# prs-eth/PCAccumulation

Measured on AMD Instinct MI355X. Metric: LiDAR-frames/sec (5-frame seq, 160k pts) fwd+bwd, higher is better.
Workload: dtype mixed

## Files before the change

include/pcacc.h:

```cpp
#ifndef PCACC_H_
#define PCACC_H_

#include <stddef.h>
#include <stdint.h>

#ifdef __cplusplus
extern "C" {
#endif

#define PCACC_OK 0
#define PCACC_E_ARG (-1)
#define PCACC_E_WORKSPACE (-2)
#define PCACC_E_LAUNCH (-3)

#define PCACC_F32 0
#define PCACC_BF16 1

const char *pcacc_target(void);

int pcacc_cat2_rows(const void *a, int32_t a_row_bytes, const void *b, int32_t b_row_bytes, int64_t rows, void *out, void *stream);

int pcacc_reload_switches(void);

int pcacc_voxelize_workspace_bytes(int64_t n, int nx, int ny, int nz, int nt, size_t *bytes );
// ... 278 lines not shown
                              float *db, int32_t n_img, int32_t frames, int32_t dt, int32_t h, int32_t w, int32_t c_in, int32_t c_out,
                              void *workspace, size_t workspace_bytes, void *stream);
int pcacc_upconv2x2_split_prepare_weights(const float *w, int32_t c_in, int32_t c_up, const int64_t *strides , uint16_t *out_fwd,
                                          float *scale_fwd, uint16_t *out_bwd, float *scale_bwd, void *stream);
int pcacc_upconv2x2_split_supported(int32_t h, int32_t w, int32_t c_in, int32_t c_up);

int pcacc_upconv2x2_bf16_supported(int32_t c_in, int32_t c_up);
int pcacc_upconv2x2_bf16_prepare_weights(const float *w, int32_t c_in, int32_t c_up, const int64_t *strides , uint16_t *out_fwd,
                                         uint16_t *out_bwd, void *stream);
int pcacc_upconv2x2_bf16(const uint16_t *in, const uint16_t *wp, const float *bias, uint16_t *out, int32_t n_img, int32_t h, int32_t w,
                         int32_t c_in, int32_t c_up, int32_t direction, int32_t in_pitch, int32_t out_pitch, void *stream);
int pcacc_upconv2x2_bf16_wgrad_workspace_bytes(int32_t n_img, int32_t h, int32_t w, int32_t c_in, int32_t c_up, size_t *bytes);
int pcacc_upconv2x2_bf16_wgrad(const uint16_t *dy, int32_t dy_pitch, const uint16_t *x, int32_t x_pitch, float *dw, const int64_t *dw_strides ,
                               float *db, int32_t n_img, int32_t h, int32_t w, int32_t c_in, int32_t c_up, void *workspace, size_t workspace_bytes,
                               void *stream);

int pcacc_prepare_weights_batch(const int64_t *jobs, int32_t n_jobs, int32_t total_blocks, void *stream);
int pcacc_upconv2x2_split(const float *in, const float *in_amax, const uint16_t *wp, const float *wscale, const float *bias, float *out,
                          float *out_amax, int32_t n_img, int32_t h, int32_t w, int32_t c_in, int32_t c_up, int32_t direction, void *stream);
int pcacc_upconv2x2_split_dual(const float *in, const float *in_amax, const uint16_t *wp, const float *wscale, const float *bias, float *out,
                               float *out_amax, uint16_t *out16, int32_t n_img, int32_t h, int32_t w, int32_t c_in, int32_t c_up,
                               int32_t out_pitch, void *stream);
int pcacc_upconv2x2_wgrad_split_workspace_bytes(int32_t n_img, int32_t h, int32_t w, int32_t c_in, int32_t c_up, size_t *bytes );
int pcacc_upconv2x2_wgrad_split(const float *dy, const float *dy_amax, const float *x, const float *x_amax, float *dw, float *db4, int32_t n_img,
                                int32_t h, int32_t w, int32_t c_in, int32_t c_up, void *workspace, size_t workspace_bytes, void *stream);
int pcacc_head_conv3x3_supported(int32_t c_in, int32_t c_out);
int pcacc_head_conv3x3_forward(const void *x, int32_t x_dtype, const float *w, const int64_t *w_strides , const float *bias, float *y,
                               int32_t n_img, int32_t h, int32_t wd, int32_t c_in, int32_t c_out, void *stream);
int pcacc_head_conv3x3_dgrad(const float *dy, const float *w, const int64_t *w_strides , void *dx, int32_t dx_dtype, int32_t n_img,
                             int32_t h, int32_t wd, int32_t c_in, int32_t c_out, void *stream);
int pcacc_head_conv3x3_wgrad_workspace_bytes(int32_t n_img, int32_t h, int32_t wd, int32_t c_in, int32_t c_out, size_t *bytes );
int pcacc_head_conv3x3_wgrad(const float *dy, const void *x, int32_t x_dtype, float *dw, float *db, int32_t n_img, int32_t h, int32_t wd,
                             int32_t c_in, int32_t c_out, void *workspace, size_t workspace_bytes, void *stream);
int pcacc_rows_linear_split(const float *x, const float *x_amax, const float *in_mask, const float *w, const float *bias,
                            const float *residual, const float *out_mask, float *y, float *y_amax, int64_t rows, int32_t k, int32_t n,
                            int32_t flags, void *stream);
int pcacc_rows_linear_split_dual(const float *x, const float *x_amax, const float *in_mask, const float *w, const float *bias,
                                 const float *residual, const float *out_mask, float *y, uint16_t *y16, float *y_amax, int64_t rows, int32_t k,
                                 int32_t n, int32_t flags, void *stream);
int pcacc_rows_linear_cat_split(const float *xa, const float *xa_amax, const float *xb, const float *xb_amax, const int32_t *b_index,
                                int32_t ka, const float *in_mask, const float *w, const float *bias, const float *residual,
                                const float *out_mask_a, const float *out_mask_b, float *y, float *y2, int32_t na, float *y_amax, int64_t rows,
                                int32_t k, int32_t n, int32_t flags, void *stream);
int pcacc_rows_wgrad_split_workspace_bytes(int64_t rows, int32_t k, int32_t n, size_t *bytes );
int pcacc_rows_wgrad_split(const float *dy, const float *dy_amax, const float *dy_mask, const float *x, const float *x_amax, int32_t x_relu,
                           int64_t rows, int32_t k, int32_t n, float *dw_aug, void *workspace, size_t workspace_bytes, void *stream);
int pcacc_rows_wgrad_cat_split(const float *dy, const float *dy_amax, const float *dy_mask, const float *xa, const float *xa_amax,
                               const float *xb, const float *xb_amax, const int32_t *b_index, int32_t ka, int32_t x_relu, int64_t rows,
                               int32_t k, int32_t n, float *dw_aug, void *workspace, size_t workspace_bytes, void *stream);
int pcacc_conv3x3_wgrad_workspace_bytes(int32_t n_img, int32_t h, int32_t w, int32_t c_in, int32_t c_out, size_t *bytes );
int pcacc_conv3x3_wgrad_bf16(const uint16_t *dy, const uint16_t *x, float *dw, int32_t n_img, int32_t frames, int32_t dt,
                             int32_t h, int32_t w, int32_t c_in, int32_t c_out, void *workspace, size_t workspace_bytes,
                             void *stream);

int pcacc_prep_points(const double *points, const double *tsfm12, const double *noise, double noise_scale, double scale,
                      double crop_xy, double z_min, double z_max, int32_t remove_ground, double ground_z, int64_t m,
                      double *out_points, uint8_t *keep, void *stream);

int pcacc_seg_loss_workspace_bytes(int64_t n, size_t *bytes );
int pcacc_seg_loss_forward(const void *logits, int logits_dtype, int64_t plane, const int64_t *labels, const int64_t *rows,
                           int64_t n, float *out_loss, double *out_metric, float *lovasz_grad, float *saved,
                           void *workspace, size_t workspace_bytes, void *stream);
int pcacc_seg_loss_backward(const void *logits, int logits_dtype, int64_t plane, const int64_t *labels, const int64_t *rows,
                            int64_t n, int64_t n_total, const float *lovasz_grad, const float *saved, const float *grad_bce,
                            const float *grad_lovasz, void *grad_logits, void *stream);

int pcacc_offset_loss_workspace_bytes(int64_t m, int64_t k, size_t *bytes );
int pcacc_offset_loss_forward(const float *points, const int64_t *time_indice, const int64_t *inst_labels,
                              const int64_t *label_base, const float *ego_motion, const float *inst_motion, int32_t n_frames,
                              int64_t n, int64_t k, const float *transformed_points, const float *offset_est,
                              const int64_t *rows, int64_t m, float *out, float *offset_gt, void *workspace,
                              size_t workspace_bytes, void *stream);
int pcacc_offset_loss_backward(const float *offset_gt, const float *offset_est, const int64_t *rows, int64_t m, int64_t n,
                               const float *grad_norm, const float *grad_dir, float *grad_est, void *stream);

int pcacc_frames_max(const void *x, int dtype, int64_t n_seq, int32_t frames, int64_t plane, void *out, uint8_t *arg, void *stream);
int pcacc_frames_max_backward(const void *grad_out, const uint8_t *arg, int dtype, int64_t n_seq, int32_t frames, int64_t plane,
                              void *grad_x, void *stream);

int pcacc_bn_rows_workspace_bytes(int64_t rows, int32_t c, size_t *bytes );
int pcacc_bn_rows_forward(const void *x, int dtype, int64_t rows, int32_t c, const float *gamma, const float *beta, float eps,
                          float momentum, float *running_mean, float *running_var, void *y, float *save_mean,
                          float *save_invstd, void *workspace, size_t workspace_bytes, void *stream);
int pcacc_bn_rows_backward(const void *grad_y, const void *x, int dtype, int64_t rows, int32_t c, const float *gamma,
                           const float *save_mean, const float *save_invstd, void *grad_x, float *grad_gamma, float *grad_beta,
                           void *workspace, size_t workspace_bytes, void *stream);

int pcacc_bn_relu_rows_forward(const void *x, int dtype, int64_t rows, int32_t c, const float *gamma, const float *beta, float eps,
                               float momentum, float *running_mean, float *running_var, void *y, float *save_mean, float *save_invstd,
                               void *workspace, size_t workspace_bytes, void *stream);
int pcacc_bn_relu_rows_backward(const void *grad_y, const void *x, int dtype, int64_t rows, int32_t c, const float *gamma, const float *beta,
                                const float *save_mean, const float *save_invstd, void *grad_x, float *grad_gamma, float *grad_beta,
                                void *workspace, size_t workspace_bytes, void *stream);
int pcacc_bn_rows_forward_dual(const float *x, int64_t rows, int32_t c, const float *gamma, const float *beta, float eps, float momentum,
                               float *running_mean, float *running_var, int32_t relu, float *y, uint16_t *y16, float *y_amax, float *save_mean,
                               float *save_invstd, void *workspace, size_t workspace_bytes, void *stream);

int pcacc_bn_rows_backward_m(const void *grad_y, const void *x, int dtype, int64_t rows, int32_t c, const float *gamma, const float *beta,
                             int32_t relu, const float *save_mean, const float *save_invstd, void *grad_x, float *grad_x_amax, float *grad_gamma,
                             float *grad_beta, void *workspace, size_t workspace_bytes, void *stream);

int pcacc_pfn_block_forward(const uint16_t *xa, const uint16_t *pooled, const int32_t *p2v, const float *w0, const float *b0,
                            const float *ws, const float *w1, const float *b1, uint16_t *out, uint16_t *relu_h, int64_t rows, void *stream);
int pcacc_pfn_block_backward_workspace_bytes(int64_t rows, size_t *bytes );
int pcacc_pfn_block_backward(const uint16_t *xa, const uint16_t *pooled, const int32_t *p2v, const uint16_t *relu_h,
                             const uint16_t *grad_out, const float *w0, const float *ws, const float *w1, uint16_t *grad_xa,
// ... 58 lines not shown
```

pcaccumulation_amd/csrc/conv.hip:

```cpp
#include "common.h"

#define CV_TH 8
#define CV_TW 32
#define CV_PW (CV_TW + 2)
#define CV_PH (CV_TH + 2)
#define CV_THREADS 256

__global__ __launch_bounds__(256) void conv_prepare_weights_kernel(const float *__restrict__ w, int o, int i, int kt, int transpose,
                                                                   uint16_t *__restrict__ out)
{
    const int taps = kt * 9;
    const int64_t total = (int64_t)taps * o * i;
    for (int64_t e = (int64_t)blockIdx.x * 256 + threadIdx.x; e < total; e += (int64_t)gridDim.x * 256) {
        const int op = transpose ? i : o, ip = transpose ? o : i;
        const int ci = (int)(e % ip);
        const int co = (int)((e / ip) % op);
        const int tap = (int)(e / ((int64_t)ip * op));
        const int src_tap = transpose ? (taps - 1 - tap) : tap;
        const int so = transpose ? ci : co, si = transpose ? co : ci;
        out[e] = f32_to_bf16(w[((int64_t)so * i + si) * taps + src_tap]);
    }
}

extern "C" int pcacc_conv3x3_prepare_weights(const float *w, int32_t c_out, int32_t c_in, int32_t kt, int32_t transpose,
                                             uint16_t *out, void *stream)
{
    if (!w || !out || c_out < 1 || c_in < 1 || (kt != 1 && kt != 3)) return PCACC_E_ARG;
    const int64_t total = (int64_t)kt * 9 * c_out * c_in;
    hipLaunchKernelGGL(conv_prepare_weights_kernel, dim3(pcacc_grid(total, 256)), dim3(256), 0, pcacc_stream(stream), w, c_out, c_in,
                       kt, transpose, out);
    PCACC_CHECK_LAUNCH();
    return 0;
}

struct ConvWStrides { int64_t o, i, t, y, x; };

__global__ __launch_bounds__(256) void conv_prepare_weights_pair_kernel(const float *__restrict__ w, int o, int i, int kt, ConvWStrides st,
                                                                        uint16_t *__restrict__ out_fwd, uint16_t *__restrict__ out_bwd)
{
    const int taps = kt * 9;
    const int64_t total = (int64_t)taps * o * i;
    for (int64_t e = (int64_t)blockIdx.x * 256 + threadIdx.x; e < 2 * total; e += (int64_t)gridDim.x * 256) {
        const bool transpose = e >= total;
        const int64_t r = transpose ? e - total : e;
        const int op = transpose ? i : o, ip = transpose ? o : i;
        const int ci = (int)(r % ip);
        const int co = (int)((r / ip) % op);
        const int tap = (int)(r / ((int64_t)ip * op));
        const int src_tap = transpose ? (taps - 1 - tap) : tap;
        const int so = transpose ? ci : co, si = transpose ? co : ci;
        const int ft = src_tap / 9, fy = (src_tap % 9) / 3, fx = src_tap % 3;
        const uint16_t v = f32_to_bf16(w[so * st.o + si * st.i + ft * st.t + fy * st.y + fx * st.x]);
        (transpose ? out_bwd : out_fwd)[r] = v;
// ... 617 lines not shown
                const int tap = grp + j * TG;
                if (tap < 9) {
                    const uint16_t *pb = sx + ((ry + tap / 3) * CV_PW + xb + tap % 3 + tr_row) * XS + it * 32 + tr_col;
                    cv_frag bf;
                    bf.h[0] = __builtin_amdgcn_ds_read_tr16_b64_v4i16((pcacc_s16x4 __attribute__((address_space(3))) *)pb);
                    bf.h[1] = __builtin_amdgcn_ds_read_tr16_b64_v4i16((pcacc_s16x4 __attribute__((address_space(3))) *)(pb + 4 * XS));
                    acc[j] = __builtin_amdgcn_mfma_f32_32x32x16_bf16(af.v, bf.v, acc[j], 0, 0, 0);
                }
            }
        }
    }
    float *mine = partial + (int64_t)blockIdx.x * (CO * 9 * CI + CO);
#pragma unroll
    for (int j = 0; j < NT; ++j) {
        const int tap = grp + j * TG;
        if (tap < 9)
#pragma unroll
            for (int r = 0; r < 16; ++r) {
                const int co = ct * 32 + (r & 3) + 8 * (r >> 2) + 4 * lh;
                mine[((int64_t)co * 9 + tap) * CI + it * 32 + lp] = acc[j][r];
            }
    }
    if (grp != 0) return;
    bsum += __shfl_xor(bsum, 32, 64);
    if (it == 0 && lh == 0) mine[CO * 9 * CI + ct * 32 + lp] = bsum;
}

template <int EL>
__global__ __launch_bounds__(1024) void conv_wgrad_reduce_kernel(const float *__restrict__ partial, int n_parts, int elems, float *__restrict__ out)
{
    pcacc_reduce_partials<EL>(partial, n_parts, elems, [&](int e, float v) { out[e] = v; });
}

static int conv_wgrad_grid(int c_in, int c_out, int64_t n_tiles)
{
    const size_t lds = (size_t)(CV_TH * CV_TW * pcacc_tr_stride(c_out) + CV_PH * CV_PW * pcacc_tr_stride(c_in)) * sizeof(uint16_t);
    int per_cu = (int)((160 * 1024) / lds);
    per_cu = per_cu > 3 ? 3 : (per_cu < 1 ? 1 : per_cu);
    int64_t slots = (int64_t)PCACC_CUS * per_cu / 8;
    const int64_t need = (n_tiles + 7) / 8;
    if (slots > need) slots = need;
    if (slots < 1) slots = 1;
    return (int)(8 * slots);
}

extern "C" int pcacc_conv3x3_wgrad_workspace_bytes(int32_t n_img, int32_t h, int32_t w, int32_t c_in, int32_t c_out, size_t *bytes)
{
    if (!bytes || n_img < 1 || h < 1 || w < 1 || (c_in != 32 && c_in != 64) || (c_out != 32 && c_out != 64)) return PCACC_E_ARG;
    const int64_t n_tiles = (int64_t)n_img * ((h + CV_TH - 1) / CV_TH) * ((w + CV_TW - 1) / CV_TW);
    *bytes = (size_t)conv_wgrad_grid(c_in, c_out, n_tiles) * (c_out * 9 * c_in + c_out) * sizeof(float);
    return 0;
}

extern "C" int pcacc_conv3x3_wgrad_bf16(const uint16_t *dy, const uint16_t *x, float *dw, int32_t n_img, int32_t frames, int32_t dt,
                                        int32_t h, int32_t w, int32_t c_in, int32_t c_out, void *workspace, size_t workspace_bytes,
                                        void *stream)
{
    if (!dy || !x || !dw || !workspace || n_img < 1 || h < 1 || w < 1 || frames < 1 || n_img % frames || dt < -1 || dt > 1)
        return PCACC_E_ARG;
    if ((c_in != 32 && c_in != 64) || (c_out != 32 && c_out != 64)) return PCACC_E_ARG;
    hipStream_t st = pcacc_stream(stream);
    const int tiles_x = (w + CV_TW - 1) / CV_TW, tiles_y = (h + CV_TH - 1) / CV_TH;
    const int64_t n_tiles = (int64_t)n_img * tiles_y * tiles_x;
    if (n_tiles > 0x7fffffff || !PCACC_WALK_OK(n_img, frames, tiles_y, tiles_x)) return PCACC_E_ARG;
    const int grid = conv_wgrad_grid(c_in, c_out, n_tiles);
    const int elems = c_out * 9 * c_in + c_out;
    if (workspace_bytes < (size_t)grid * elems * sizeof(float)) return PCACC_E_WORKSPACE;
    const size_t lds = (size_t)(CV_TH * CV_TW * pcacc_tr_stride(c_out) + CV_PH * CV_PW * pcacc_tr_stride(c_in)) * sizeof(uint16_t);
    float *partial = reinterpret_cast<float *>(workspace);
#define CV_WG(COT, CIT)                                                                                                              \
    do {                                                                                                                             \
        auto kern = conv3x3_wgrad_kernel<COT, CIT>;                                                                                  \
        if (lds > 64 * 1024 && hipFuncSetAttribute(reinterpret_cast<const void *>(kern), hipFuncAttributeMaxDynamicSharedMemorySize, \
                                                   (int)lds) != hipSuccess)                                                          \
            return PCACC_E_LAUNCH;                                                                                                   \
        hipLaunchKernelGGL(kern, dim3(grid), dim3(CV_THREADS), lds, st, dy, x, partial, n_img, frames, dt, h, w, tiles_x, tiles_y, dw); \
    } while (0)
    if (c_out == 32 && c_in == 32) CV_WG(1, 1);
    else if (c_out == 32 && c_in == 64) CV_WG(1, 2);
    else if (c_out == 64 && c_in == 32) CV_WG(2, 1);
    else CV_WG(2, 2);
#undef CV_WG
    if (pcacc_reduce_el(elems) == 64) conv_wgrad_reduce_kernel<64><<<(elems + 63) / 64, 1024, 0, st>>>(partial, grid, elems, dw);
    else conv_wgrad_reduce_kernel<16><<<(elems + 15) / 16, 1024, 0, st>>>(partial, grid, elems, dw);
    PCACC_CHECK_LAUNCH();
    return 0;
}
```

pcaccumulation_amd/native.py:

```python
import ctypes
import os
import re

import torch

_HERE = os.path.dirname(os.path.abspath(__file__))
LIB_PATH = os.environ.get('PCACC_LIB') or os.path.join(_HERE, 'csrc', 'libpcacc_hip.so')

F32, BF16 = 0, 1
_ERR = {-1: 'PCACC_E_ARG', -2: 'PCACC_E_WORKSPACE', -3: 'PCACC_E_LAUNCH'}

_lib = None


class NativeError(RuntimeError):
    pass


_CTYPES = {'int': ctypes.c_int, 'int32_t': ctypes.c_int, 'int64_t': ctypes.c_int64, 'uint64_t': ctypes.c_uint64, 'size_t': ctypes.c_size_t,
           'float': ctypes.c_float, 'double': ctypes.c_double}


def _prototypes():
    text = re.sub(r'/\*.*?\*/', '', open(os.path.join(_HERE, os.pardir, 'include', 'pcacc.h')).read(), flags=re.S)
# ... 746 lines not shown
        raise NativeError('conv3x3: weights prepared for %d input channels, input has %d' % (wc_in, c_in))
    out = torch.empty((n_img, h, w, c_out), dtype=torch.bfloat16, device=x_rows.device)
    if out_mask is not None:
        if bias is not None or relu or mask is not None or tuple(out_mask.shape) != tuple(out.shape):
            raise NativeError('conv3x3: out_mask goes with no bias / relu / input mask and has the shape of the result')
        _check(lib().pcacc_conv3x3_outmask_bf16(_dev(x_rows, torch.bfloat16, 'x'), _dev(wp, torch.bfloat16, 'wp'),
                                                _dev(out_mask, torch.bfloat16, 'out_mask'), _dev(out), int(n_img), int(frames), int(h), int(w),
                                                int(c_in), int(c_out), taps // 9, _stream()), 'conv3x3_outmask')
        return out
    if mask is not None and mask.shape != x_rows.shape:
        raise NativeError('conv3x3: mask shape %s != input shape %s' % (tuple(mask.shape), tuple(x_rows.shape)))
    _check(lib().pcacc_conv3x3_masked_bf16(_dev(x_rows, torch.bfloat16, 'x'), _dev(mask, torch.bfloat16, 'mask') if mask is not None else None,
                                           _dev(wp, torch.bfloat16, 'wp'), _dev(bias, torch.float32, 'bias') if bias is not None else None,
                                           _dev(out), int(n_img), int(frames), int(h), int(w), int(c_in), int(c_out), taps // 9,
                                           1 if relu else 0, _stream()), 'conv3x3')
    return out


def sample_subsets(counts, k, seed):
    d = counts.shape[0]
    out = torch.empty((d, k), dtype=torch.int64, device=counts.device)
    _check(lib().pcacc_sample_subsets(_dev(counts, torch.int32, 'counts'), int(d), int(k), int(seed) & (2 ** 64 - 1), _dev(out), _stream()), 'sample_subsets')
    return out


def conv3x3_wgrad_supported(c_in, c_out):
    return c_in in (32, 64) and c_out in (32, 64)


def conv3x3_wgrad(dy_rows, x_rows, frames=1, dt=0):
    n_img, h, w, c_out = dy_rows.shape
    c_in = x_rows.shape[3]
    dw = torch.empty((c_out * 9 * c_in + c_out,), dtype=torch.float32, device=dy_rows.device)
    ws = _workspace(lib().pcacc_conv3x3_wgrad_workspace_bytes, dy_rows.device, int(n_img), int(h), int(w), int(c_in), int(c_out))
    _check(lib().pcacc_conv3x3_wgrad_bf16(_dev(dy_rows, torch.bfloat16, 'dy'), _dev(x_rows, torch.bfloat16, 'x'), _dev(dw), int(n_img),
                                          int(frames), int(dt), int(h), int(w), int(c_in), int(c_out), _dev(ws), ws.numel(), _stream()), 'conv3x3_wgrad')
    return dw[:c_out * 9 * c_in].view(c_out, 9, c_in), dw[c_out * 9 * c_in:]


def conv3x3_wgrad_deep_supported(h, w, c_in, c_out):
    return bool(lib().pcacc_conv3x3_wgrad_deep_supported(int(h), int(w), int(c_in), int(c_out)))


def conv3x3_wgrad_deep(dy_rows, x_rows, mask=None):
    n_img, h, w, c_out = dy_rows.shape
    c_in = x_rows.shape[3]
    dw = torch.empty((c_out, 9, c_in), dtype=torch.float32, device=dy_rows.device)
    db = torch.empty((c_out,), dtype=torch.float32, device=dy_rows.device)
    ws = _workspace(lib().pcacc_conv3x3_wgrad_deep_workspace_bytes, dy_rows.device, int(n_img), int(h), int(w), int(c_in), int(c_out))
    _check(lib().pcacc_conv3x3_wgrad_deep_bf16(_dev(dy_rows, torch.bfloat16, 'dy'), _dev(mask, torch.bfloat16, 'mask') if mask is not None else None,
                                               _dev(x_rows, torch.bfloat16, 'x'), _dev(dw), _dev(db),
                                               int(n_img), int(h), int(w), int(c_in), int(c_out), _dev(ws), ws.numel(), _stream()), 'conv3x3_wgrad_deep')
    return dw, db


def absmax256(t):
    out = torch.empty((256,), dtype=torch.float32, device=t.device)
    if not t.is_cuda or t.dtype != torch.float32:
        raise NativeError('absmax256: float32 GPU tensor expected, got %s on %s' % (t.dtype, t.device))
    if not (t.is_contiguous() or torch.ops.aten.is_non_overlapping_and_dense(t)):
        t = t.contiguous()
    _check(lib().pcacc_absmax256(ctypes.c_void_p(t.data_ptr()), t.numel(), _dev(out), _stream()), 'absmax256')
    return out


_ZERO_POOL = {}


def _zero256(device):
    key = (device.type, device.index, torch.cuda.current_stream(device).cuda_stream if device.type == 'cuda' else 0)
    blk = _ZERO_POOL.get(key)
    if blk is None or blk[1] >= blk[0].shape[0]:
        blk = [torch.zeros((128, 256), dtype=torch.float32, device=device), 0]
        _ZERO_POOL[key] = blk
    row = blk[0][blk[1]]
    blk[1] += 1
    return row


def conv3x3_split_supported(h, w, c_in, c_out):
    return bool(lib().pcacc_conv3x3_split_supported(int(h), int(w), int(c_in), int(c_out)))


def conv3x3_split_prepare_weights(weight):
    o, i = weight.shape[0], weight.shape[1]
    kt = 3 if weight.dim() == 5 else 1
    if not weight.is_cuda or weight.dtype != torch.float32:
        raise NativeError('conv3x3_split_prepare_weights: weight must be a float32 GPU tensor')
    fwd = torch.empty((2, kt * 9, o, i), dtype=torch.float16, device=weight.device)
    bwd = torch.empty((2, kt * 9, i, o), dtype=torch.float16, device=weight.device)
    sf = torch.empty((o,), dtype=torch.float32, device=weight.device)
    sb = torch.empty((i,), dtype=torch.float32, device=weight.device)
    strides = (ctypes.c_int64 * weight.dim())(*weight.stride())
    _check(lib().pcacc_conv3x3_split_prepare_weights(ctypes.c_void_p(weight.data_ptr()), int(o), int(i), kt, strides, _dev(fwd), _dev(sf),
                                                     _dev(bwd), _dev(sb), _stream()), 'conv3x3_split_prepare_weights')
    return (fwd, sf), (bwd, sb)


def conv3x3_split(x_rows, wps, bias, frames, relu, mask=None, amax=None, want_amax=False, out_mask=None, want_bf16=False):
    wp, wscale = wps
    n_img, h, w, c_in = x_rows.shape
    _, taps, c_out, wc_in = wp.shape
    if wc_in != c_in:
        raise NativeError('conv3x3_split: weights prepared for %d input channels, input has %d' % (wc_in, c_in))
    if mask is not None and mask.shape != x_rows.shape:
        raise NativeError('conv3x3_split: mask shape %s != input shape %s' % (tuple(mask.shape), tuple(x_rows.shape)))
# ... 885 lines not shown
```

pcaccumulation_amd/ops.py:

```python
import weakref

import os

import torch

from . import native


class PillarIndex(object):

    def __init__(self, coordinates, point_to_voxel_map, batch_size, input_shape, cell_order=False):
        nx, ny, nz, nt = (int(v) for v in input_shape[:4])
        self.nx, self.ny, self.nt, self.batch_size = nx, ny, nt, int(batch_size)
        self.m = int(coordinates.shape[0])
        self.n_cells = self.batch_size * nt * ny * nx
        self.cells_per_frame = ny * nx
        coords = coordinates.contiguous()
        if coords.dtype not in (torch.float64, torch.int32):
            coords = coords.to(torch.float64)
        self.cell, self.cell2pillar = native.cell_index(coords, nx, ny, nt, self.batch_size)
        self.coordinates, self.perm, self._frames = coordinates, None, None
        p2v = point_to_voxel_map
        if p2v is not None:
            p2v = (p2v[:, 0] if p2v.dim() == 2 else p2v).to(torch.int32)
# ... 1110 lines not shown
            self.entries.clear()
        self.put(weight, fwd, bwd)
        return fwd, bwd


def _detached_f32(weight):
    w = weight.detach()
    return w if w.dtype == torch.float32 else w.float()


_FORMS = {
    0: _PreparedForms(0, lambda w: native.conv3x3_split_prepare_weights(_detached_f32(w))),
    1: _PreparedForms(1, lambda w: native.upconv2x2_split_prepare_weights(w.detach())),
    2: _PreparedForms(2, lambda w: native.conv3x3_prepare_weights_pair(_detached_f32(w))),
    3: _PreparedForms(3, lambda w: native.upconv2x2_bf16_prepare_weights(w.detach())),
}


def prepared_conv_weights(weight):
    return _FORMS[2].forms(weight)


def prepared_conv_weights_split(weight):
    return _FORMS[0].forms(weight)


def prepared_upconv_weights_split(weight):
    return _FORMS[1].forms(weight)


def prepared_upconv_weights_bf16(weight):
    return _FORMS[3].forms(weight)


class _Conv3x3(torch.autograd.Function):

    @staticmethod
    def forward(ctx, x_rows, weight, bias, frames, relu, premasked=False, input_relu=False):
        y = native.conv3x3(x_rows, prepared_conv_weights(weight)[0], bias.detach().float() if bias is not None else None, frames, relu)
        ctx.save_for_backward(x_rows, weight, y if relu and not premasked else None)
        ctx.meta = (frames, relu and not premasked, bias is not None, bool(input_relu))
        return y

    @staticmethod
    def backward(ctx, gy):
        x_rows, weight, y = ctx.saved_tensors
        frames, relu, has_bias, input_relu = ctx.meta
        gy = gy.contiguous()
        gx = gw = gb = None
        kt = 3 if weight.dim() == 5 else 1
        o, i = weight.shape[0], weight.shape[1]
        h, w = x_rows.shape[1], x_rows.shape[2]
        need_w = ctx.needs_input_grad[1] or (has_bias and ctx.needs_input_grad[2])
        lib_dgrad = ctx.needs_input_grad[0] and kt == 1 and not conv3x3_preferred(o, i, h, w)
        deep_w = need_w and kt == 1 and not native.conv3x3_wgrad_supported(i, o) and native.conv3x3_wgrad_deep_supported(h, w, i, o)
        deep_d = ctx.needs_input_grad[0] and kt == 1 and o > 64 and native.conv3x3_deep_supported(h, w, o, i)
        mask = y if relu and (deep_w or not need_w) and (deep_d or not ctx.needs_input_grad[0]) else None
        if relu and mask is None:
            gy = torch.ops.aten.threshold_backward(gy, y, 0)
        gx_masked = False
        if ctx.needs_input_grad[0] and not lib_dgrad:
            if input_relu and mask is None and native.conv3x3_outmask_supported(h, w, o, i, kt):
                gx = native.conv3x3(gy, prepared_conv_weights(weight)[1], None, frames, False, out_mask=x_rows)
                gx_masked = True
            else:
                gx = native.conv3x3(gy, prepared_conv_weights(weight)[1], None, frames, False, mask=mask)
        if need_w and native.conv3x3_wgrad_supported(i, o):
            if kt == 3:
                parts = [native.conv3x3_wgrad(gy, x_rows, frames, dt) for dt in (-1, 0, 1)]
                gw = torch.stack([p[0].view(o, 3, 3, i) for p in parts], dim=1).permute(0, 4, 1, 2, 3)
                gb = parts[1][1]
            else:
                gw, gb = native.conv3x3_wgrad(gy, x_rows)
                gw = gw.view(o, 3, 3, i).permute(0, 3, 1, 2)
            gw = gw.to(weight.dtype)
            gb = gb.clone() if has_bias and ctx.needs_input_grad[2] else None
            need_w = False
        elif deep_w:
            gw, gb = native.conv3x3_wgrad_deep(gy, x_rows, mask=mask)
            gw = gw.view(o, 3, 3, i).permute(0, 3, 1, 2).to(weight.dtype)
            gb = gb if has_bias and ctx.needs_input_grad[2] else None
            need_w = False
        if need_w or lib_dgrad:
            xin = _stack_frames(x_rows, frames) if kt == 3 else x_rows
            w2 = weight.detach().permute(0, 2, 1, 3, 4).reshape(o, 3 * i, 3, 3) if kt == 3 else weight.detach()
            gx2, gw2, gb2 = torch.ops.aten.convolution_backward(
                gy.permute(0, 3, 1, 2), xin.permute(0, 3, 1, 2), w2.to(torch.bfloat16).contiguous(memory_format=torch.channels_last),
                [o] if has_bias else None, [1, 1], [1, 1], [1, 1], False, [0, 0], 1, [lib_dgrad, need_w, has_bias and need_w])
            if lib_dgrad:
                gx = gx2.permute(0, 2, 3, 1).contiguous()
            if need_w:
                gw = gw2.float()
                if kt == 3:
                    gw = gw.reshape(o, 3, i, 3, 3).permute(0, 2, 1, 3, 4)
                gw = gw.reshape(weight.shape)
                gb = gb2.float() if has_bias else None
        if input_relu and gx is not None and not gx_masked:
            gx = torch.ops.aten.threshold_backward(gx, x_rows, 0)
        return gx, gw, gb, None, None, None, None


class _Conv3x3Split(torch.autograd.Function):

    @staticmethod
    def forward(ctx, x_rows, weight, bias, frames, relu, premasked=False, input_relu=False):
        x_amax = amax_of(x_rows)
# ... 64 lines not shown
    @staticmethod
    def backward(ctx, gy):
        return _Conv3x3.backward(ctx, gy)[:3] + (None, None, None, None)


def conv3x3_cat(a, b, conv, relu=False, premasked=False):
    if (_MIXED and a.is_cuda and a.dtype == torch.bfloat16 and b.dtype == torch.bfloat16 and a.dim() == 4 and a.shape[1] % 32 == 0
            and b.shape[1] % 32 == 0 and os.environ.get('PCACC_CONV_CAT', '1') != '0' and conv3x3_native(a.new_empty((0, a.shape[1] + b.shape[1]) + tuple(a.shape[2:])), conv) == 'mixed'):
        ar, br = a.permute(0, 2, 3, 1), b.permute(0, 2, 3, 1)
        a32, b32 = twin(ar), twin(br)
        if ar.is_contiguous() and br.is_contiguous() and a32.is_contiguous() and b32.is_contiguous():
            x16 = _cat2(ar, br, -1)
            if _POISON:
                with torch.no_grad():
                    x16.fill_(float('nan'))
            return _Conv3x3CatMixed.apply(x16, conv.weight, conv.bias, bool(relu), bool(premasked), a32, b32).permute(0, 3, 1, 2)
    return conv3x3(cat_maps((a, b), 1), conv, relu=relu, premasked=premasked)


class _UpConv2x2Split(torch.autograd.Function):

    @staticmethod
    def forward(ctx, x_rows, weight, bias):
        x_amax = amax_of(x_rows)
        y, y_amax = native.upconv2x2_split(x_rows, x_amax, prepared_upconv_weights_split(weight)[0], bias.detach() if bias is not None else None, 0)
        set_amax_tag(y, y_amax)
        ctx.save_for_backward(x_rows, weight, x_amax)
        ctx.has_bias = bias is not None
        return y

    @staticmethod
    def backward(ctx, gy):
        x_rows, weight, x_amax = ctx.saved_tensors
        gy = dense(gy)
        if gy.dtype != torch.float32:
            gy = gy.float()
        g_amax = amax_of(gy)
        gx = gw = gb = None
        if ctx.needs_input_grad[0]:
            gx, gx_amax = native.upconv2x2_split(gy, g_amax, prepared_upconv_weights_split(weight)[1], None, 1)
            set_amax_tag(gx, gx_amax)
        if ctx.needs_input_grad[1] or (ctx.has_bias and ctx.needs_input_grad[2]):
            gw, gb = native.upconv2x2_wgrad_split(gy, g_amax, x_rows, x_amax)
            gw = gw.to(weight.dtype)
            gb = gb if ctx.has_bias and ctx.needs_input_grad[2] else None
        return gx, gw, gb


def _upconv_bf16_backward(ctx, gy, x_rows, weight):
    c_in, c_up = weight.shape[0], weight.shape[1]
    if gy.dtype != torch.bfloat16:
        gy = gy.to(torch.bfloat16)
    if native.upconv2x2_bf16_supported(c_in, c_up) and weight.dtype == torch.float32 and os.environ.get('PCACC_UPCONV_BF16', '1') != '0':
        gx = native.upconv2x2_bf16(gy, prepared_upconv_weights_bf16(weight)[1], None, 1) if ctx.needs_input_grad[0] else None
        gw = gb = None
        if ctx.needs_input_grad[1] or (ctx.has_bias and ctx.needs_input_grad[2]):
            gw, gb = native.upconv2x2_bf16_wgrad(gy, x_rows, want_bias=ctx.has_bias and ctx.needs_input_grad[2], like=weight)
        return gx, gw, gb
    gy = gy.contiguous()
    w16 = weight.detach().to(torch.bfloat16).contiguous(memory_format=torch.channels_last)
    gx, gw, _ = torch.ops.aten.convolution_backward(
        gy.permute(0, 3, 1, 2), x_rows.permute(0, 3, 1, 2), w16, None, [2, 2], [0, 0], [1, 1], True, [0, 0], 1,
        [ctx.needs_input_grad[0], ctx.needs_input_grad[1], False])
    gb = gy.reshape(-1, gy.shape[-1]).sum(0, dtype=torch.float32) if ctx.has_bias and ctx.needs_input_grad[2] else None
    if gx is not None:
        gx = gx.permute(0, 2, 3, 1).contiguous()
    return gx, (gw.float().contiguous(memory_format=torch.channels_last) if gw is not None else None), gb


class _UpConv2x2Bf16(torch.autograd.Function):

    @staticmethod
    def forward(ctx, x_rows, weight, bias):
        ctx.save_for_backward(x_rows, weight)
        ctx.has_bias = bias is not None
        return native.upconv2x2_bf16(x_rows, prepared_upconv_weights_bf16(weight)[0], bias.detach().float() if bias is not None else None, 0)

    @staticmethod
    def backward(ctx, gy):
        x_rows, weight = ctx.saved_tensors
        return _upconv_bf16_backward(ctx, gy, x_rows, weight)


class _UpConv2x2Mixed(torch.autograd.Function):

    @staticmethod
    def forward(ctx, x_rows, weight, bias):
        x32 = twin(x_rows)
        y32, y_amax, y16 = native.upconv2x2_split(x32, amax_of(x32), prepared_upconv_weights_split(weight)[0], bias.detach() if bias is not None else None, 0,
                                                  want_bf16=True)
        set_amax_tag(y32, y_amax)
        ctx.save_for_backward(x_rows, weight)
        ctx.has_bias = bias is not None
        return shadow(y32, y16)

    @staticmethod
    def backward(ctx, gy):
        x_rows, weight = ctx.saved_tensors
        return _upconv_bf16_backward(ctx, gy, x_rows, weight)


class _UpConvCatMixed(torch.autograd.Function):

    @staticmethod
    def forward(ctx, x_rows, skip_rows, weight, bias):
        x32, s32 = twin(x_rows), twin(skip_rows)
# ... 551 lines not shown
```

Measured before the change: 676.9.

## Add fused native backward entry points for conv3x3 and upconv2x2

```diff
diff --git a/include/pcacc.h b/include/pcacc.h
--- a/include/pcacc.h
+++ b/include/pcacc.h
@@ -354,6 +354,16 @@
 int pcacc_conv3x3_wgrad_bf16(const uint16_t *dy, const uint16_t *x, float *dw, int32_t n_img, int32_t frames, int32_t dt,
                              int32_t h, int32_t w, int32_t c_in, int32_t c_out, void *workspace, size_t workspace_bytes,
                              void *stream);
+int pcacc_conv3x3_backward_supported(int32_t h, int32_t w, int32_t c_in, int32_t c_out, int32_t kt, int32_t flags);
+int pcacc_conv3x3_backward_workspace_bytes(int32_t n_img, int32_t h, int32_t w, int32_t c_in, int32_t c_out, int32_t kt, int32_t flags,
+                                           size_t *bytes );
+int pcacc_conv3x3_backward_bf16(const uint16_t *dy, const uint16_t *y, const uint16_t *x, const uint16_t *wp_dgrad, uint16_t *gx, float *gw,
+                                float *gb, int32_t n_img, int32_t frames, int32_t h, int32_t w, int32_t c_in, int32_t c_out, int32_t kt,
+                                int32_t flags, void *workspace, size_t workspace_bytes, void *stream);
+int pcacc_upconv2x2_backward_workspace_bytes(int32_t n_img, int32_t h, int32_t w, int32_t c_in, int32_t c_up, size_t *bytes );
+int pcacc_upconv2x2_backward_bf16(const uint16_t *dy, int32_t dy_pitch, const uint16_t *x, int32_t x_pitch, const uint16_t *wp_dgrad, uint16_t *gx,
+                                  float *gw, const int64_t *gw_strides , float *gb, int32_t n_img, int32_t h, int32_t w, int32_t c_in,
+                                  int32_t c_up, void *workspace, size_t workspace_bytes, void *stream);
 
 int pcacc_prep_points(const double *points, const double *tsfm12, const double *noise, double noise_scale, double scale,
                       double crop_xy, double z_min, double z_max, int32_t remove_ground, double ground_z, int64_t m,
diff --git a/pcaccumulation_amd/csrc/conv.hip b/pcaccumulation_amd/csrc/conv.hip
--- a/pcaccumulation_amd/csrc/conv.hip
+++ b/pcaccumulation_amd/csrc/conv.hip
@@ -1,4 +1,5 @@
 #include "common.h"
+#include "conv_internal.h"
 
 #define CV_TH 8
 #define CV_TW 32
@@ -722,35 +723,54 @@
     return 0;
 }
 
-extern "C" int pcacc_conv3x3_wgrad_bf16(const uint16_t *dy, const uint16_t *x, float *dw, int32_t n_img, int32_t frames, int32_t dt,
-                                        int32_t h, int32_t w, int32_t c_in, int32_t c_out, void *workspace, size_t workspace_bytes,
-                                        void *stream)
-{
-    if (!dy || !x || !dw || !workspace || n_img < 1 || h < 1 || w < 1 || frames < 1 || n_img % frames || dt < -1 || dt > 1)
+int conv_wgrad_mfma_grid(int n_img, int h, int w, int c_in, int c_out)
+{
+    const int64_t n_tiles = (int64_t)n_img * ((h + CV_TH - 1) / CV_TH) * ((w + CV_TW - 1) / CV_TW);
+    return conv_wgrad_grid(c_in, c_out, n_tiles);
+}
+
+int conv_wgrad_mfma_partials(const uint16_t *dy, const uint16_t *x, float *partial, float *dw_zero, int n_img, int frames, int dt, int h, int w,
+                             int c_in, int c_out, hipStream_t st)
+{
+    if (!dy || !x || !dw_zero || !partial || n_img < 1 || h < 1 || w < 1 || frames < 1 || n_img % frames || dt < -1 || dt > 1)
         return PCACC_E_ARG;
     if ((c_in != 32 && c_in != 64) || (c_out != 32 && c_out != 64)) return PCACC_E_ARG;
-    hipStream_t st = pcacc_stream(stream);
     const int tiles_x = (w + CV_TW - 1) / CV_TW, tiles_y = (h + CV_TH - 1) / CV_TH;
     const int64_t n_tiles = (int64_t)n_img * tiles_y * tiles_x;
     if (n_tiles > 0x7fffffff || !PCACC_WALK_OK(n_img, frames, tiles_y, tiles_x)) return PCACC_E_ARG;
     const int grid = conv_wgrad_grid(c_in, c_out, n_tiles);
-    const int elems = c_out * 9 * c_in + c_out;
-    if (workspace_bytes < (size_t)grid * elems * sizeof(float)) return PCACC_E_WORKSPACE;
     const size_t lds = (size_t)(CV_TH * CV_TW * pcacc_tr_stride(c_out) + CV_PH * CV_PW * pcacc_tr_stride(c_in)) * sizeof(uint16_t);
-    float *partial = reinterpret_cast<float *>(workspace);
 #define CV_WG(COT, CIT)                                                                                                              \
     do {                                                                                                                             \
         auto kern = conv3x3_wgrad_kernel<COT, CIT>;                                                                                  \
         if (lds > 64 * 1024 && hipFuncSetAttribute(reinterpret_cast<const void *>(kern), hipFuncAttributeMaxDynamicSharedMemorySize, \
                                                    (int)lds) != hipSuccess)                                                          \
             return PCACC_E_LAUNCH;                                                                                                   \
-        hipLaunchKernelGGL(kern, dim3(grid), dim3(CV_THREADS), lds, st, dy, x, partial, n_img, frames, dt, h, w, tiles_x, tiles_y, dw); \
+        hipLaunchKernelGGL(kern, dim3(grid), dim3(CV_THREADS), lds, st, dy, x, partial, n_img, frames, dt, h, w, tiles_x, tiles_y, dw_zero); \
     } while (0)
     if (c_out == 32 && c_in == 32) CV_WG(1, 1);
     else if (c_out == 32 && c_in == 64) CV_WG(1, 2);
     else if (c_out == 64 && c_in == 32) CV_WG(2, 1);
     else CV_WG(2, 2);
 #undef CV_WG
+    PCACC_CHECK_LAUNCH();
+    return 0;
+}
+
+extern "C" int pcacc_conv3x3_wgrad_bf16(const uint16_t *dy, const uint16_t *x, float *dw, int32_t n_img, int32_t frames, int32_t dt,
+                                        int32_t h, int32_t w, int32_t c_in, int32_t c_out, void *workspace, size_t workspace_bytes,
+                                        void *stream)
+{
+    if (!dy || !x || !dw || !workspace || n_img < 1 || h < 1 || w < 1 || frames < 1 || n_img % frames || dt < -1 || dt > 1)
+        return PCACC_E_ARG;
+    if ((c_in != 32 && c_in != 64) || (c_out != 32 && c_out != 64)) return PCACC_E_ARG;
+    hipStream_t st = pcacc_stream(stream);
+    const int grid = conv_wgrad_mfma_grid(n_img, h, w, c_in, c_out);
+    const int elems = c_out * 9 * c_in + c_out;
+    if (workspace_bytes < (size_t)grid * elems * sizeof(float)) return PCACC_E_WORKSPACE;
+    float *partial = reinterpret_cast<float *>(workspace);
+    const int rc = conv_wgrad_mfma_partials(dy, x, partial, dw, n_img, frames, dt, h, w, c_in, c_out, st);
+    if (rc != 0) return rc;
     if (pcacc_reduce_el(elems) == 64) conv_wgrad_reduce_kernel<64><<<(elems + 63) / 64, 1024, 0, st>>>(partial, grid, elems, dw);
     else conv_wgrad_reduce_kernel<16><<<(elems + 15) / 16, 1024, 0, st>>>(partial, grid, elems, dw);
     PCACC_CHECK_LAUNCH();
diff --git a/pcaccumulation_amd/csrc/conv_backward.hip b/pcaccumulation_amd/csrc/conv_backward.hip
--- /dev/null
+++ b/pcaccumulation_amd/csrc/conv_backward.hip
@@ -0,0 +1,166 @@
+#include "common.h"
+#include "conv_internal.h"
+
+#define CB_WANT_GX 1
+#define CB_WANT_GW 2
+#define CB_WANT_GB 4
+#define CB_INPUT_RELU 8
+#define CB_RELU 16
+
+__global__ __launch_bounds__(256) void conv_relu_mask_kernel(const uint4 *v, const uint4 *__restrict__ m, uint4 *out, int64_t n8)
+{
+    for (int64_t i = (int64_t)blockIdx.x * 256 + threadIdx.x; i < n8; i += (int64_t)gridDim.x * 256) {
+        const uint4 a = v[i], b = m[i];
+        out[i] = make_uint4(conv_mask2(a.x, b.x), conv_mask2(a.y, b.y), conv_mask2(a.z, b.z), conv_mask2(a.w, b.w));
+    }
+}
+
+static int conv_relu_mask(const uint16_t *v, const uint16_t *m, uint16_t *out, int64_t n, hipStream_t st)
+{
+    const int64_t n8 = n / 8;
+    hipLaunchKernelGGL(conv_relu_mask_kernel, dim3(pcacc_grid(n8, 256)), dim3(256), 0, st, reinterpret_cast<const uint4 *>(v),
+                       reinterpret_cast<const uint4 *>(m), reinterpret_cast<uint4 *>(out), n8);
+    PCACC_CHECK_LAUNCH();
+    return 0;
+}
+
+template <int EL>
+__global__ __launch_bounds__(1024) void conv_backward_reduce_kernel(const float *__restrict__ partial, int n_parts, int elems, int kt, int row,
+                                                                    int n_w, float *__restrict__ gw, float *__restrict__ gb)
+{
+    const int t = blockIdx.y;
+    pcacc_reduce_partials<EL>(partial + (int64_t)t * n_parts * elems, n_parts, elems, [&](int e, float v) {
+        if (e < n_w) {
+            const int co = e / row;
+            gw[((int64_t)co * kt + t) * row + (e - co * row)] = v;
+        } else if (gb && t == kt / 2) {
+            gb[e - n_w] = v;
+        }
+    });
+}
+
+struct ConvBackwardPlan {
+    bool need_w, want_gx, mfma_w, deep_w, deep_d, staged, mask_pass, outmask;
+    size_t dy_bytes, partial_bytes, scratch_bytes, deep_bytes;
+    int grid, elems;
+};
+
+static bool conv_backward_plan(int n_img, int h, int w, int c_in, int c_out, int kt, int flags, ConvBackwardPlan *p)
+{
+    if (n_img < 1 || h < 1 || w < 1 || (kt != 1 && kt != 3) || c_in < 32 || c_out < 32 || c_in % 32 || c_out % 32) return false;
+    p->want_gx = (flags & CB_WANT_GX) != 0;
+    p->need_w = (flags & (CB_WANT_GW | CB_WANT_GB)) != 0;
+    const bool relu = (flags & CB_RELU) != 0, input_relu = (flags & CB_INPUT_RELU) != 0;
+    if (p->want_gx && kt == 1 && c_out > 64 && !pcacc_conv3x3_deep_supported(h, w, c_out, c_in)) return false;
+    p->mfma_w = p->need_w && (c_in == 32 || c_in == 64) && (c_out == 32 || c_out == 64);
+    p->deep_w = p->need_w && kt == 1 && !p->mfma_w && pcacc_conv3x3_wgrad_deep_supported(h, w, c_in, c_out);
+    if (p->need_w && !p->mfma_w && !p->deep_w) return false;
+    p->deep_d = p->want_gx && kt == 1 && c_out > 64 && pcacc_conv3x3_deep_supported(h, w, c_out, c_in);
+    p->staged = relu && (p->deep_w || !p->need_w) && (p->deep_d || !p->want_gx);
+    p->mask_pass = relu && !p->staged;
+    p->outmask = p->want_gx && input_relu && !p->staged && pcacc_conv3x3_outmask_supported(h, w, c_out, c_in, kt);
+    p->dy_bytes = p->mask_pass ? pcacc_align((size_t)n_img * h * w * c_out * sizeof(uint16_t)) : 0;
+    p->partial_bytes = p->scratch_bytes = p->deep_bytes = 0;
+    p->grid = 0;
+    p->elems = c_out * 9 * c_in + c_out;
+    if (p->mfma_w) {
+        p->grid = conv_wgrad_mfma_grid(n_img, h, w, c_in, c_out);
+        p->partial_bytes = pcacc_align((size_t)kt * p->grid * p->elems * sizeof(float));
+        p->scratch_bytes = pcacc_align((size_t)p->elems * sizeof(float));
+    } else if (p->deep_w) {
+        if (pcacc_conv3x3_wgrad_deep_workspace_bytes(n_img, h, w, c_in, c_out, &p->deep_bytes) != 0) return false;
+        p->deep_bytes = pcacc_align(p->deep_bytes);
+        p->scratch_bytes = pcacc_align((size_t)c_out * sizeof(float));
+    }
+    return true;
+}
+
+extern "C" int pcacc_conv3x3_backward_supported(int32_t h, int32_t w, int32_t c_in, int32_t c_out, int32_t kt, int32_t flags)
+{
+    ConvBackwardPlan p;
+    return conv_backward_plan(1, h, w, c_in, c_out, kt, flags, &p) ? 1 : 0;
+}
+
+extern "C" int pcacc_conv3x3_backward_workspace_bytes(int32_t n_img, int32_t h, int32_t w, int32_t c_in, int32_t c_out, int32_t kt, int32_t flags,
+                                                      size_t *bytes)
+{
+    ConvBackwardPlan p;
+    if (!bytes || !conv_backward_plan(n_img, h, w, c_in, c_out, kt, flags, &p)) return PCACC_E_ARG;
+    *bytes = p.dy_bytes + p.partial_bytes + p.deep_bytes + p.scratch_bytes;
+    return 0;
+}
+
+extern "C" int pcacc_conv3x3_backward_bf16(const uint16_t *dy, const uint16_t *y, const uint16_t *x, const uint16_t *wp_dgrad, uint16_t *gx,
+                                           float *gw, float *gb, int32_t n_img, int32_t frames, int32_t h, int32_t w, int32_t c_in,
+                                           int32_t c_out, int32_t kt, int32_t flags, void *workspace, size_t workspace_bytes, void *stream)
+{
+    ConvBackwardPlan p;
+    if (flags & ~(CB_WANT_GX | CB_WANT_GW | CB_WANT_GB | CB_INPUT_RELU | CB_RELU)) return PCACC_E_ARG;
+    flags = (flags & ~CB_RELU) | (y ? CB_RELU : 0);
+    if (!dy || !x || frames < 1 || n_img < 1 || n_img % frames || !conv_backward_plan(n_img, h, w, c_in, c_out, kt, flags, &p)) return PCACC_E_ARG;
+    if ((p.want_gx && (!gx || !wp_dgrad)) || (p.need_w && !gw) || ((flags & CB_WANT_GB) && !gb)) return PCACC_E_ARG;
+    if (((uintptr_t)dy | (uintptr_t)y | (uintptr_t)x | (uintptr_t)gx | (uintptr_t)workspace) & 15) return PCACC_E_ARG;
+    const size_t need = p.dy_bytes + p.partial_bytes + p.deep_bytes + p.scratch_bytes;
+    if (need && (!workspace || workspace_bytes < need)) return PCACC_E_WORKSPACE;
+    hipStream_t st = pcacc_stream(stream);
+    char *ws = static_cast<char *>(workspace);
+    uint16_t *dy_masked = reinterpret_cast<uint16_t *>(ws);
+    char *w_part = ws + p.dy_bytes;
+    float *scratch = reinterpret_cast<float *>(w_part + p.partial_bytes + p.deep_bytes);
+    const int64_t n_dy = (int64_t)n_img * h * w * c_out, n_x = (int64_t)n_img * h * w * c_in;
+    int rc;
+    if (p.mask_pass) {
+        if ((rc = conv_relu_mask(dy, y, dy_masked, n_dy, st)) != 0) return rc;
+        dy = dy_masked;
+    }
+    const uint16_t *stage_mask = p.staged ? y : nullptr;
+    if (p.want_gx) {
+        if (p.outmask) {
+            rc = pcacc_conv3x3_outmask_bf16(dy, wp_dgrad, x, gx, n_img, frames, h, w, c_out, c_in, kt, stream);
+        } else {
+            rc = pcacc_conv3x3_masked_bf16(dy, stage_mask, wp_dgrad, nullptr, gx, n_img, frames, h, w, c_out, c_in, kt, 0, stream);
+            if (rc == 0 && (flags & CB_INPUT_RELU)) rc = conv_relu_mask(gx, x, gx, n_x, st);
+        }
+        if (rc != 0) return rc;
+    }
+    if (p.mfma_w) {
+        float *partial = reinterpret_cast<float *>(w_part);
+        for (int t = 0; t < kt; ++t) {
+            rc = conv_wgrad_mfma_partials(dy, x, partial + (size_t)t * p.grid * p.elems, scratch, n_img, kt == 3 ? frames : 1, kt == 3 ? t - 1 : 0,
+                                          h, w, c_in, c_out, st);
+            if (rc != 0) return rc;
+        }
+        const int n_w = c_out * 9 * c_in;
+        float *gb_out = (flags & CB_WANT_GB) ? gb : nullptr;
+        if (pcacc_reduce_el(p.elems) == 64)
+            hipLaunchKernelGGL(conv_backward_reduce_kernel<64>, dim3((p.elems + 63) / 64, kt), dim3(1024), 0, st, partial, p.grid, p.elems, kt, 9 * c_in,
+                               n_w, gw, gb_out);
+        else
+            hipLaunchKernelGGL(conv_backward_reduce_kernel<16>, dim3((p.elems + 15) / 16, kt), dim3(1024), 0, st, partial, p.grid, p.elems, kt, 9 * c_in,
+                               n_w, gw, gb_out);
+        PCACC_CHECK_LAUNCH();
+    } else if (p.deep_w) {
+        rc = pcacc_conv3x3_wgrad_deep_bf16(dy, stage_mask, x, gw, (flags & CB_WANT_GB) ? gb : scratch, n_img, h, w, c_in, c_out, w_part, p.deep_bytes,
+                                           stream);
+        if (rc != 0) return rc;
+    }
+    return 0;
+}
+
+extern "C" int pcacc_upconv2x2_backward_workspace_bytes(int32_t n_img, int32_t h, int32_t w, int32_t c_in, int32_t c_up, size_t *bytes)
+{
+    return pcacc_upconv2x2_bf16_wgrad_workspace_bytes(n_img, h, w, c_in, c_up, bytes);
+}
+
+extern "C" int pcacc_upconv2x2_backward_bf16(const uint16_t *dy, int32_t dy_pitch, const uint16_t *x, int32_t x_pitch, const uint16_t *wp_dgrad,
+                                             uint16_t *gx, float *gw, const int64_t *gw_strides, float *gb, int32_t n_img, int32_t h, int32_t w,
+                                             int32_t c_in, int32_t c_up, void *workspace, size_t workspace_bytes, void *stream)
+{
+    int rc;
+    if (!gx && !gw) return PCACC_E_ARG;
+    if (gx && (rc = pcacc_upconv2x2_bf16(dy, wp_dgrad, nullptr, gx, n_img, h, w, c_in, c_up, 1, dy_pitch, c_in, stream)) != 0) return rc;
+    if (gw && (rc = pcacc_upconv2x2_bf16_wgrad(dy, dy_pitch, x, x_pitch, gw, gw_strides, gb, n_img, h, w, c_in, c_up, workspace, workspace_bytes,
+                                                stream)) != 0)
+        return rc;
+    return 0;
+}
diff --git a/pcaccumulation_amd/csrc/conv_internal.h b/pcaccumulation_amd/csrc/conv_internal.h
--- /dev/null
+++ b/pcaccumulation_amd/csrc/conv_internal.h
@@ -0,0 +1,6 @@
+#pragma once
+#include "common.h"
+
+int conv_wgrad_mfma_grid(int n_img, int h, int w, int c_in, int c_out);
+int conv_wgrad_mfma_partials(const uint16_t *dy, const uint16_t *x, float *partial, float *dw_zero, int n_img, int frames, int dt, int h, int w,
+                             int c_in, int c_out, hipStream_t st);
diff --git a/pcaccumulation_amd/native.py b/pcaccumulation_amd/native.py
--- a/pcaccumulation_amd/native.py
+++ b/pcaccumulation_amd/native.py
@@ -822,6 +822,68 @@
                                                _dev(x_rows, torch.bfloat16, 'x'), _dev(dw), _dev(db),
                                                int(n_img), int(h), int(w), int(c_in), int(c_out), _dev(ws), ws.numel(), _stream()), 'conv3x3_wgrad_deep')
     return dw, db
+
+
+CB_GX, CB_GW, CB_GB, CB_INPUT_RELU, CB_RELU = 1, 2, 4, 8, 16
+_CB_SUPPORTED = {}
+
+
+def conv3x3_backward_supported(h, w, c_in, c_out, kt, flags):
+    key = (h, w, c_in, c_out, kt, flags)
+    hit = _CB_SUPPORTED.get(key)
+    if hit is None:
+        hit = _CB_SUPPORTED[key] = bool(lib().pcacc_conv3x3_backward_supported(int(h), int(w), int(c_in), int(c_out), int(kt), int(flags)))
+    return hit
+
+
+def conv3x3_backward(dy_rows, y, x_rows, wp_dgrad, frames, kt, flags):
+    n_img, h, w, c_out = dy_rows.shape
+    c_in = x_rows.shape[3]
+    dev = dy_rows.device
+    flags = (flags & ~CB_RELU) | (CB_RELU if y is not None else 0)
+    gx = torch.empty((n_img, h, w, c_in), dtype=torch.bfloat16, device=dev) if flags & CB_GX else None
+    gw = gb = flat = None
+    if flags & (CB_GW | CB_GB):
+        flat = torch.empty((c_out, kt, 3, 3, c_in), dtype=torch.float32, device=dev)
+        gw = flat.permute(0, 4, 1, 2, 3) if kt == 3 else flat.view(c_out, 3, 3, c_in).permute(0, 3, 1, 2)
+        if flags & CB_GB:
+            gb = torch.empty((c_out,), dtype=torch.float32, device=dev)
+    ws = _workspace(lib().pcacc_conv3x3_backward_workspace_bytes, dev, int(n_img), int(h), int(w), int(c_in), int(c_out), int(kt), int(flags))
+    _check(lib().pcacc_conv3x3_backward_bf16(_dev(dy_rows, torch.bfloat16, 'dy'), _dev(y, torch.bfloat16, 'y') if y is not None else None,
+                                             _dev(x_rows, torch.bfloat16, 'x'), _dev(wp_dgrad, torch.bfloat16, 'wp') if gx is not None else None,
+                                             _dev(gx) if gx is not None else None, _dev(flat) if flat is not None else None,
+                                             _dev(gb) if gb is not None else None, int(n_img), int(frames), int(h), int(w), int(c_in), int(c_out),
+                                             int(kt), int(flags), _dev(ws), ws.numel(), _stream()), 'conv3x3_backward')
+    return gx, gw, gb
+
+
+def upconv2x2_backward(dy_rows, x_rows, wp_dgrad, want_gx=True, want_gw=True, want_bias=True, like=None):
+    n, h, w, c_in = x_rows.shape
+    c_up = dy_rows.shape[3]
+    dp, xp = _rows_pitch(dy_rows, 'dy'), _rows_pitch(x_rows, 'x')
+    if dp is None:
+        dy_rows, dp = dy_rows.contiguous(), c_up
+    if xp is None:
+        x_rows, xp = x_rows.contiguous(), c_in
+    if dy_rows.dtype != torch.bfloat16 or x_rows.dtype != torch.bfloat16 or tuple(dy_rows.shape[:3]) != (n, 2 * h, 2 * w) or not dy_rows.is_cuda:
+        raise NativeError('upconv2x2_backward: bf16 GPU rows [n,2h,2w,c_up] and [n,h,w,c_in] expected')
+    dev = x_rows.device
+    gx = torch.empty((n, h, w, c_in), dtype=torch.bfloat16, device=dev) if want_gx else None
+    dw = db = dws = None
+    if want_gw:
+        if like is not None and tuple(like.shape) == (c_in, c_up, 2, 2):
+            dw = torch.empty_strided(like.shape, like.stride(), dtype=torch.float32, device=dev)
+        else:
+            dw = torch.empty((c_in, c_up, 2, 2), dtype=torch.float32, device=dev)
+        dws = (ctypes.c_int64 * 4)(*dw.stride())
+        db = torch.empty((c_up,), dtype=torch.float32, device=dev) if want_bias else None
+    ws = _workspace(lib().pcacc_upconv2x2_backward_workspace_bytes, dev, int(n), int(h), int(w), int(c_in), int(c_up))
+    _check(lib().pcacc_upconv2x2_backward_bf16(ctypes.c_void_p(dy_rows.data_ptr()), int(dp), ctypes.c_void_p(x_rows.data_ptr()), int(xp),
+                                               _dev(wp_dgrad, torch.bfloat16, 'wp') if gx is not None else None,
+                                               _dev(gx) if gx is not None else None, ctypes.c_void_p(dw.data_ptr()) if dw is not None else None,
+                                               dws, _dev(db) if db is not None else None, int(n), int(h), int(w), int(c_in), int(c_up), _dev(ws),
+                                               ws.numel(), _stream()), 'upconv2x2_backward')
+    return gx, dw, db
 
 
 def absmax256(t):
diff --git a/pcaccumulation_amd/ops.py b/pcaccumulation_amd/ops.py
--- a/pcaccumulation_amd/ops.py
+++ b/pcaccumulation_amd/ops.py
@@ -1186,6 +1186,14 @@
         o, i = weight.shape[0], weight.shape[1]
         h, w = x_rows.shape[1], x_rows.shape[2]
         need_w = ctx.needs_input_grad[1] or (has_bias and ctx.needs_input_grad[2])
+        if os.environ.get('PCACC_CONV_BWD_ENTRY', '1') != '0':
+            flags = ((native.CB_GX if ctx.needs_input_grad[0] else 0) | (native.CB_GW if need_w else 0)
+                     | (native.CB_GB if has_bias and ctx.needs_input_grad[2] else 0) | (native.CB_INPUT_RELU if input_relu else 0)
+                     | (native.CB_RELU if relu else 0))
+            if native.conv3x3_backward_supported(h, w, i, o, kt, flags):
+                gx, gw, gb = native.conv3x3_backward(gy, y if relu else None, x_rows, prepared_conv_weights(weight)[1] if flags & native.CB_GX else None,
+                                                     frames, kt, flags)
+                return gx, (gw.to(weight.dtype) if gw is not None else None), gb, None, None, None, None
         lib_dgrad = ctx.needs_input_grad[0] and kt == 1 and not conv3x3_preferred(o, i, h, w)
         deep_w = need_w and kt == 1 and not native.conv3x3_wgrad_supported(i, o) and native.conv3x3_wgrad_deep_supported(h, w, i, o)
         deep_d = ctx.needs_input_grad[0] and kt == 1 and o > 64 and native.conv3x3_deep_supported(h, w, o, i)
@@ -1356,6 +1364,10 @@
     if gy.dtype != torch.bfloat16:
         gy = gy.to(torch.bfloat16)
     if native.upconv2x2_bf16_supported(c_in, c_up) and weight.dtype == torch.float32 and os.environ.get('PCACC_UPCONV_BF16', '1') != '0':
+        want_w = ctx.needs_input_grad[1] or (ctx.has_bias and ctx.needs_input_grad[2])
+        if os.environ.get('PCACC_CONV_BWD_ENTRY', '1') != '0' and (ctx.needs_input_grad[0] or want_w):
+            return native.upconv2x2_backward(gy, x_rows, prepared_upconv_weights_bf16(weight)[1] if ctx.needs_input_grad[0] else None,
+                                             want_gx=ctx.needs_input_grad[0], want_gw=want_w, want_bias=ctx.has_bias and ctx.needs_input_grad[2], like=weight)
         gx = native.upconv2x2_bf16(gy, prepared_upconv_weights_bf16(weight)[1], None, 1) if ctx.needs_input_grad[0] else None
         gw = gb = None
         if ctx.needs_input_grad[1] or (ctx.has_bias and ctx.needs_input_grad[2]):
```

New measurement: 677.8, median of 2. No clear change (+0.1%).
